# DJjjjhao/FIRA-ICSE

Measured on NVIDIA H100. Metric: train_commits_per_sec, higher is better.
Workload: dtype bf16

## Files before the change

fira_icse_b200/csrc/gcn_fused.cu:

```cuda
#include "tc_common.cuh"
#include "fira_b200.h"

namespace {

using namespace tc;

constexpr int D = 256;
constexpr int TM = 128;
constexpr int N_CONSUMER = 256;
constexpr int N_GATHER = 4;
constexpr int THREADS = N_CONSUMER + N_GATHER * 32;
constexpr int EC = 1024;
constexpr uint32_t B_BYTES = D * D * 2;
constexpr uint32_t A_BYTES = TM * D * 2;
constexpr uint32_t OFF_A = B_BYTES, OFF_ROWPTR = OFF_A + A_BYTES, OFF_COL = OFF_ROWPTR + 544, OFF_VAL = OFF_COL + EC * 4,
                   OFF_RS = OFF_VAL + EC * 4, SMEM_BYTES = OFF_RS + 4 * TM * 4;
constexpr int GATHER_BAR = 1;

struct Params {
  const int* rowptr; const int* col; const float* val;
  const __nv_bfloat16* x;
  long R;
  const float* bias; const float* c1; const float* gamma; const float* beta;
  __nv_bfloat16* z; __nv_bfloat16* outA; __nv_bfloat16* outB; long split;
  float* mean; float* rstd;
  float p_drop; uint64_t seed; const uint64_t* seed_ctr; uint32_t stream_id;
  const __nv_bfloat16* addend; __nv_bfloat16* agg_out; __nv_bfloat16* y;
};

__device__ __forceinline__ void tile_range(long R, int cta, int ncta, int t, long& r0, int& rows, int& ntiles) {
  const long rpc = (R + ncta - 1) / ncta;
  const long lo = (long)cta * rpc;
  const long hi = lo + rpc < R ? lo + rpc : R;
  const long n = hi > lo ? hi - lo : 0;
  ntiles = (int)((n + TM - 1) / TM);
  if (ntiles == 0) { r0 = 0; rows = 0; return; }
  long chunk = (n + ntiles - 1) / ntiles;
  chunk = (chunk + 7) & ~7L;
  if (chunk > TM) chunk = TM;
  r0 = lo + (long)t * chunk;
  const long e = r0 + chunk < hi ? r0 + chunk : hi;
  rows = (int)(e > r0 ? e - r0 : 0);
}

__device__ __forceinline__ uint4 pack8(const float* v) {
  uint4 r;
  __nv_bfloat162* h = reinterpret_cast<__nv_bfloat162*>(&r);
#pragma unroll
  for (int i = 0; i < 4; ++i) h[i] = __floats2bfloat162_rn(v[2 * i], v[2 * i + 1]);
  return r;
}
__device__ __forceinline__ void unpack8(const uint4& raw, float* v) {
  const __nv_bfloat162* h = reinterpret_cast<const __nv_bfloat162*>(&raw);
#pragma unroll
  for (int i = 0; i < 4; ++i) { const float2 f = __bfloat1622float2(h[i]); v[2 * i] = f.x; v[2 * i + 1] = f.y; }
}

template <int MODE>
__global__ void __launch_bounds__(THREADS, 1) gcn_fused_kernel(const __grid_constant__ CUtensorMap tmW, Params p) {
  extern __shared__ unsigned char smem_raw[];
  __shared__ __align__(8) unsigned long long b_full, a_full, a_empty;
  const uint32_t base = (smem_addr(smem_raw) + 1023u) & ~1023u;
  unsigned char* sm = smem_raw + (base - smem_addr(smem_raw));
  const int warp = threadIdx.x >> 5, lane = threadIdx.x & 31;
  const int cta = blockIdx.x, ncta = gridDim.x;
  long r0_; int rows_, ntiles;
  tile_range(p.R, cta, ncta, 0, r0_, rows_, ntiles);

  if (threadIdx.x == 0) {
    mbar_init(smem_addr(&b_full), 1);
    mbar_init(smem_addr(&a_full), N_GATHER * 32);
    mbar_init(smem_addr(&a_empty), N_CONSUMER);
    mbar_init_fence();
    tma_prefetch_desc(&tmW);
  }
  __syncthreads();
  pdl_wait(); pdl_trigger();

  if (warp >= N_CONSUMER / 32) {
    const int gw = warp - N_CONSUMER / 32;
    const int gtid = gw * 32 + lane;
    const int q = lane >> 3, ql = lane & 7;
    int* s_rowptr = reinterpret_cast<int*>(sm + OFF_ROWPTR);
    int* s_col = reinterpret_cast<int*>(sm + OFF_COL);
    float* s_val = reinterpret_cast<float*>(sm + OFF_VAL);
    float* s_rs = reinterpret_cast<float*>(sm + OFF_RS);
    for (int t = 0; t < ntiles; ++t) {
      long r0; int rows, nt_;
      tile_range(p.R, cta, ncta, t, r0, rows, nt_);
      if (t >= 1) named_bar(GATHER_BAR, N_GATHER * 32);
      for (int i = gtid; i <= rows; i += N_GATHER * 32) s_rowptr[i] = p.rowptr[r0 + i];
      named_bar(GATHER_BAR, N_GATHER * 32);
      const int e_lo = s_rowptr[0], e_hi = s_rowptr[rows];
      const int nE = e_hi - e_lo;
      const bool staged = nE <= EC;
      if (staged)
        for (int i = gtid; i < nE; i += N_GATHER * 32) { s_col[i] = p.col[e_lo + i]; s_val[i] = p.val[e_lo + i]; }
      if (t >= 1 && gtid == 0) mbar_wait(smem_addr(&a_empty), (t - 1) & 1);
      named_bar(GATHER_BAR, N_GATHER * 32);
      const int* cp = staged ? s_col : p.col + e_lo;
      const float* vp = staged ? s_val : p.val + e_lo;
#pragma unroll 1
      for (int it = 0; it < 8; ++it) {
        const int r = gw * 32 + it * 4 + q;
        if (r < rows) {
          const int e0 = s_rowptr[r] - e_lo, e1 = s_rowptr[r + 1] - e_lo;
          float acc[4][8];
#pragma unroll
          for (int j = 0; j < 4; ++j)
#pragma unroll
            for (int i = 0; i < 8; ++i) acc[j][i] = 0.f;
          float rsum = 0.f;
          int e = e0;
          for (; e + 1 < e1; e += 2) {
            const int c0 = cp[e], c1 = cp[e + 1];
            const float w0 = vp[e], w1 = vp[e + 1];
            const uint4* s0 = reinterpret_cast<const uint4*>(p.x + (long)c0 * D + ql * 8);
            const uint4* s1 = reinterpret_cast<const uint4*>(p.x + (long)c1 * D + ql * 8);
            uint4 a[4], b[4];
#pragma unroll
            for (int j = 0; j < 4; ++j) a[j] = __ldg(s0 + j * 8);
#pragma unroll
            for (int j = 0; j < 4; ++j) b[j] = __ldg(s1 + j * 8);
            rsum += w0 + w1;
#pragma unroll
            for (int j = 0; j < 4; ++j) {
              float f[8];
              unpack8(a[j], f);
#pragma unroll
              for (int i = 0; i < 8; ++i) acc[j][i] = fmaf(w0, f[i], acc[j][i]);
              unpack8(b[j], f);
#pragma unroll
              for (int i = 0; i < 8; ++i) acc[j][i] = fmaf(w1, f[i], acc[j][i]);
            }
          }
          if (e < e1) {
            const int c0 = cp[e];
            const float w0 = vp[e];
            const uint4* s0 = reinterpret_cast<const uint4*>(p.x + (long)c0 * D + ql * 8);
            uint4 a[4];
#pragma unroll
            for (int j = 0; j < 4; ++j) a[j] = __ldg(s0 + j * 8);
            rsum += w0;
#pragma unroll
            for (int j = 0; j < 4; ++j) {
              float f[8];
              unpack8(a[j], f);
#pragma unroll
              for (int i = 0; i < 8; ++i) acc[j][i] = fmaf(w0, f[i], acc[j][i]);
            }
          }
#pragma unroll
          for (int j = 0; j < 4; ++j) {
            const uint4 v = pack8(acc[j]);
            *reinterpret_cast<uint4*>(sm + OFF_A + j * 16384 + sw128_offset(r, ql)) = v;
            if (MODE == 1) *reinterpret_cast<uint4*>(p.agg_out + (r0 + r) * D + j * 64 + ql * 8) = v;
          }
          if (MODE == 0 && ql == 0) s_rs[(t & 3) * TM + r] = rsum;
        }
      }
      fence_proxy_async();
      mbar_arrive(smem_addr(&a_full));
    }
    return;
  }

  const int wg = warp >> 2, q4 = lane & 3;
  if (threadIdx.x == 0 && ntiles > 0) {
    mbar_expect_tx(smem_addr(&b_full), B_BYTES);
#pragma unroll
    for (int kb = 0; kb < 4; ++kb) tma_load_2d(base + kb * 32768, &tmW, kb * 64, 0, smem_addr(&b_full));
  }
  if (ntiles > 0) mbar_wait(smem_addr(&b_full), 0);
  const float* s_rs = reinterpret_cast<const float*>(sm + OFF_RS);
  uint64_t seed = p.seed;
  if (MODE == 0 && p.seed_ctr) seed += *p.seed_ctr;
  const float keep_scale = (MODE == 0 && p.p_drop > 0.f) ? 1.f / (1.f - p.p_drop) : 1.f;
  const __nv_bfloat16* resid = MODE == 0 ? p.x : p.addend;
  for (int t = 0; t < ntiles; ++t) {
    long r0; int rows, nt_;
    tile_range(p.R, cta, ncta, t, r0, rows, nt_);
    float acc[D / 2];
#pragma unroll
    for (int i = 0; i < D / 2; ++i) acc[i] = 0.f;
    mbar_wait(smem_addr(&a_full), t & 1);
    wgmma_fence();
#pragma unroll
    for (int kb = 0; kb < 4; ++kb)
#pragma unroll
      for (int k = 0; k < 4; ++k)
        wgmma<D, 0, 0>(acc, make_desc(base + OFF_A + kb * 16384 + wg * 8192 + k * 32, 16, 1024),
                       make_desc(base + kb * 32768 + k * 32, 16, 1024));
    wgmma_commit();
    wgmma_wait<0>();
    reg_fence<D / 2>(acc);
    mbar_arrive(smem_addr(&a_empty));
    int tr[2];
    bool live[2];
    long grow[2];
    float rs[2], sum[2] = {0.f, 0.f}, sq[2] = {0.f, 0.f};
#pragma unroll
    for (int h = 0; h < 2; ++h) {
      tr[h] = wg * 64 + (warp & 3) * 16 + (lane >> 2) + 8 * h;
      live[h] = tr[h] < rows;
      grow[h] = r0 + tr[h];
      rs[h] = (MODE == 0 && live[h]) ? s_rs[(t & 3) * TM + tr[h]] : 0.f;
    }
#pragma unroll
    for (int j = 0; j < D / 8; ++j) {
      const int c = 8 * j + 2 * q4;
      float2 bv = make_float2(0.f, 0.f), cv = make_float2(0.f, 0.f);
      if (MODE == 0) {
        bv = __ldg(reinterpret_cast<const float2*>(p.bias + c));
        cv = __ldg(reinterpret_cast<const float2*>(p.c1 + c));
      }
#pragma unroll
      for (int h = 0; h < 2; ++h) {
        float2 hv = make_float2(0.f, 0.f);
        if (live[h] && resid != nullptr) hv = __bfloat1622float2(__ldg(reinterpret_cast<const __nv_bfloat162*>(resid + grow[h] * D + c)));
        float v0 = acc[4 * j + 2 * h], v1 = acc[4 * j + 2 * h + 1];
        if (MODE == 0) {
          v0 = fmaf(rs[h], cv.x, v0 + bv.x);
          v1 = fmaf(rs[h], cv.y, v1 + bv.y);
          const __nv_bfloat162 zb = __floats2bfloat162_rn(v0, v1);
          if (live[h]) *reinterpret_cast<__nv_bfloat162*>(p.z + grow[h] * D + c) = zb;
          const float2 zf = __bfloat1622float2(zb);
          v0 = zf.x; v1 = zf.y;
          if (p.p_drop > 0.f) {
            const uint32_t m = dropout_keep8(seed, p.stream_id, (uint64_t)grow[h] * 32 + j, p.p_drop) >> (2 * q4);
            v0 = (m & 1) ? v0 * keep_scale : 0.f;
            v1 = (m & 2) ? v1 * keep_scale : 0.f;
          }
          v0 += hv.x; v1 += hv.y;
          acc[4 * j + 2 * h] = v0; acc[4 * j + 2 * h + 1] = v1;
          sum[h] += v0 + v1;
          sq[h] = fmaf(v0, v0, fmaf(v1, v1, sq[h]));
        } else if (live[h]) {
          *reinterpret_cast<__nv_bfloat162*>(p.y + grow[h] * D + c) = __floats2bfloat162_rn(v0 + hv.x, v1 + hv.y);
        }
      }
    }
    if (MODE == 0) {
      float mean[2], rstd[2];
#pragma unroll
      for (int h = 0; h < 2; ++h) {
        sum[h] += __shfl_xor_sync(0xffffffffu, sum[h], 1);
        sum[h] += __shfl_xor_sync(0xffffffffu, sum[h], 2);
        sq[h] += __shfl_xor_sync(0xffffffffu, sq[h], 1);
        sq[h] += __shfl_xor_sync(0xffffffffu, sq[h], 2);
        mean[h] = sum[h] * (1.f / D);
        const float var = fmaxf(sq[h] * (1.f / D) - mean[h] * mean[h], 0.f);
        rstd[h] = rsqrtf(var + kLnEps);
        if (live[h] && q4 == 0 && p.mean) { p.mean[grow[h]] = mean[h]; p.rstd[grow[h]] = rstd[h]; }
      }
#pragma unroll
      for (int j = 0; j < D / 8; ++j) {
        const int c = 8 * j + 2 * q4;
        const float2 gv = __ldg(reinterpret_cast<const float2*>(p.gamma + c));
        const float2 bt = __ldg(reinterpret_cast<const float2*>(p.beta + c));
#pragma unroll
        for (int h = 0; h < 2; ++h) {
          if (!live[h]) continue;
          const float o0 = fmaf((acc[4 * j + 2 * h] - mean[h]) * rstd[h], gv.x, bt.x);
          const float o1 = fmaf((acc[4 * j + 2 * h + 1] - mean[h]) * rstd[h], gv.y, bt.y);
          __nv_bfloat16* dst = grow[h] < p.split ? p.outA : p.outB;
          *reinterpret_cast<__nv_bfloat162*>(dst + grow[h] * D + c) = __floats2bfloat162_rn(o0, o1);
        }
      }
    }
  }
}

struct Segs { int B, n0, n1, n2; };
__device__ __forceinline__ long seg_row(const Segs& s, int b, int j) {
  if (j < s.n0) return (long)b * s.n0 + j;
  if (j < s.n0 + s.n1) return (long)s.B * s.n0 + (long)b * s.n1 + (j - s.n0);
  return (long)s.B * (s.n0 + s.n1) + (long)b * s.n2 + (j - s.n0 - s.n1);
}
__device__ __forceinline__ void seg_unrow(const Segs& s, long r, int& b, int& i) {
  const long e0 = (long)s.B * s.n0, e1 = e0 + (long)s.B * s.n1;
  if (r < e0) { b = (int)(r / s.n0); i = (int)(r % s.n0); }
  else if (r < e1) { long q = r - e0; b = (int)(q / s.n1); i = s.n0 + (int)(q % s.n1); }
// ... 35 lines not shown
    const int excl = carry + (warp ? warp_tot[warp - 1] : 0) + x - v;
    if (i < n) out[i] = excl;
    __syncthreads();
    if (threadIdx.x == 1023) carry = excl + v;
    __syncthreads();
  }
  if (threadIdx.x == 0) out[n] = carry;
}

__global__ void rows_fill_kernel(const int* __restrict__ rowptr, const int* __restrict__ col, const float* __restrict__ val,
                                 Segs s, int N, const int* __restrict__ rowptr_g, int* __restrict__ col_g,
                                 float* __restrict__ val_g) {
  pdl_wait(); pdl_trigger();
  const long R = (long)s.B * N;
  const int lane = threadIdx.x & 31;
  for (long r = (long)blockIdx.x * (blockDim.x >> 5) + (threadIdx.x >> 5); r < R; r += (long)gridDim.x * (blockDim.x >> 5)) {
    int b, i; seg_unrow(s, r, b, i);
    const long g = (long)b * N + i;
    const int e0 = rowptr[g], n = rowptr[g + 1] - e0, o0 = rowptr_g[r];
    for (int k = lane; k < n; k += 32) { col_g[o0 + k] = (int)seg_row(s, b, col[e0 + k]); val_g[o0 + k] = val[e0 + k]; }
  }
}

int launch_fused(int mode, const CUtensorMap& tm, const Params& p, cudaStream_t st) {
  static_assert(SMEM_BYTES + 1024 <= 227 * 1024, "fused GCN kernel: shared-memory budget");
  const size_t smem = SMEM_BYTES + 1024;
  cudaError_t e = mode == 0
      ? cudaFuncSetAttribute(gcn_fused_kernel<0>, cudaFuncAttributeMaxDynamicSharedMemorySize, (int)smem)
      : cudaFuncSetAttribute(gcn_fused_kernel<1>, cudaFuncAttributeMaxDynamicSharedMemorySize, (int)smem);
  if (e != cudaSuccess) { fira_set_error(FIRA_ERR_CUDA, "gcn_layer attr: %s", cudaGetErrorString(e)); return FIRA_ERR_CUDA; }
  long want = (p.R + 31) / 32;
  const int grid = (int)(want < fira_num_sms() ? (want < 1 ? 1 : want) : fira_num_sms());
  if (mode == 0) launch_k(gcn_fused_kernel<0>, dim3(grid), dim3(THREADS), smem, st, tm, p);
  else launch_k(gcn_fused_kernel<1>, dim3(grid), dim3(THREADS), smem, st, tm, p);
  return FIRA_OK;
}

}

extern "C" {

int fira_csr_to_rows(const int* rowptr, const int* col, const float* val, int B, int n_code, int n_sub, int n_ast,
                     int* counts, int* rowptr_rows, int* col_rows, float* val_rows, void* stream) {
  FIRA_CHECK_ARG(rowptr && col && val && counts && rowptr_rows && col_rows && val_rows, FIRA_ERR_ARG, "csr_to_rows: null");
  FIRA_CHECK_ARG(B > 0 && n_code > 0 && n_sub >= 0 && n_ast >= 0, FIRA_ERR_SHAPE, "csr_to_rows: segments");
  Segs s{B, n_code, n_sub, n_ast};
  const int N = n_code + n_sub + n_ast;
  const long R = (long)B * N;
  cudaStream_t st = (cudaStream_t)stream;
  int grid = (int)((R + 255) / 256 < fira_num_sms() * 4 ? (R + 255) / 256 : fira_num_sms() * 4);
  launch_k(rows_count_kernel, dim3(grid), dim3(256), 0, st, rowptr, s, N, counts);
  launch_k(rows_scan_kernel, dim3(1), dim3(1024), 0, st, counts, rowptr_rows, R);
  grid = (int)((R + 7) / 8 < fira_num_sms() * 8 ? (R + 7) / 8 : fira_num_sms() * 8);
  launch_k(rows_fill_kernel, dim3(grid), dim3(256), 0, st, rowptr, col, val, s, N, rowptr_rows, col_rows, val_rows);
  FIRA_CHECK_LAUNCH("fira_csr_to_rows");
  return FIRA_OK;
}

int fira_gcn_layer_fwd(const int* rowptr_rows, const int* col_rows, const float* val_rows, const void* h,
                       const void* w_merged, const float* bias, const float* c1, const float* gamma, const float* beta,
                       void* z, void* outA, void* outB, long split, float* mean, float* rstd, long rows, int dim,
                       float p_drop, uint64_t seed, const uint64_t* seed_ctr, uint32_t stream_id, void* stream) {
  FIRA_CHECK_ARG(dim == D, FIRA_ERR_SHAPE, "gcn_layer_fwd: dim %d != 256", dim);
  FIRA_CHECK_ARG(rows > 0, FIRA_ERR_SHAPE, "gcn_layer_fwd: rows %ld", rows);
  FIRA_CHECK_ARG(rowptr_rows && col_rows && val_rows && h && w_merged && bias && c1 && gamma && beta && z && outA && outB,
                 FIRA_ERR_ARG, "gcn_layer_fwd: null argument");
  FIRA_CHECK_ARG(fira_aligned16(h) && fira_aligned16(w_merged) && fira_aligned16(z) && fira_aligned16(outA) &&
                     fira_aligned16(outB) && fira_aligned16(bias) && fira_aligned16(c1) && fira_aligned16(gamma) &&
                     fira_aligned16(beta), FIRA_ERR_ALIGN, "gcn_layer_fwd: 16-B alignment");
  FIRA_CHECK_ARG(p_drop >= 0.f && p_drop < 1.f, FIRA_ERR_ARG, "gcn_layer_fwd: p_drop %f", p_drop);
  CUtensorMap tm;
  int rc = make_map_bf16(&tm, w_merged, D, D, D, 64, D, "gcn_layer_fwd");
  if (rc) return rc;
  Params p{};
  p.rowptr = rowptr_rows; p.col = col_rows; p.val = val_rows; p.x = (const __nv_bfloat16*)h; p.R = rows;
  p.bias = bias; p.c1 = c1; p.gamma = gamma; p.beta = beta;
  p.z = (__nv_bfloat16*)z; p.outA = (__nv_bfloat16*)outA; p.outB = (__nv_bfloat16*)outB; p.split = split;
  p.mean = mean; p.rstd = rstd; p.p_drop = p_drop; p.seed = seed; p.seed_ctr = seed_ctr; p.stream_id = stream_id;
  if ((rc = launch_fused(0, tm, p, (cudaStream_t)stream))) return rc;
  FIRA_CHECK_LAUNCH("fira_gcn_layer_fwd");
  return FIRA_OK;
}

int fira_gcn_layer_bwd(const int* rowptr_rows_t, const int* col_rows_t, const float* val_rows_t, const void* d_z,
                       const void* w_merged_t, const void* d_resid, void* agg_dz, void* d_h, long rows, int dim,
                       void* stream) {
  FIRA_CHECK_ARG(dim == D, FIRA_ERR_SHAPE, "gcn_layer_bwd: dim %d != 256", dim);
  FIRA_CHECK_ARG(rows > 0, FIRA_ERR_SHAPE, "gcn_layer_bwd: rows %ld", rows);
  FIRA_CHECK_ARG(rowptr_rows_t && col_rows_t && val_rows_t && d_z && w_merged_t && agg_dz && d_h, FIRA_ERR_ARG,
                 "gcn_layer_bwd: null argument");
  FIRA_CHECK_ARG(fira_aligned16(d_z) && fira_aligned16(w_merged_t) && fira_aligned16(d_resid) && fira_aligned16(agg_dz) &&
                     fira_aligned16(d_h), FIRA_ERR_ALIGN, "gcn_layer_bwd: 16-B alignment");
  CUtensorMap tm;
  int rc = make_map_bf16(&tm, w_merged_t, D, D, D, 64, D, "gcn_layer_bwd");
  if (rc) return rc;
  Params p{};
  p.rowptr = rowptr_rows_t; p.col = col_rows_t; p.val = val_rows_t; p.x = (const __nv_bfloat16*)d_z; p.R = rows;
  p.addend = (const __nv_bfloat16*)d_resid; p.agg_out = (__nv_bfloat16*)agg_dz; p.y = (__nv_bfloat16*)d_h;
  if ((rc = launch_fused(1, tm, p, (cudaStream_t)stream))) return rc;
  FIRA_CHECK_LAUNCH("fira_gcn_layer_bwd");
  return FIRA_OK;
}

}
```

fira_icse_b200/ops.py:

```python
import ctypes
import os

import torch

from . import _lib
from . import optim as _optim
from ._lib import FIRA_BF16, FIRA_F32, call

D = 256

if hasattr(torch.autograd.graph, "set_warn_on_accumulate_grad_stream_mismatch"):
    torch.autograd.graph.set_warn_on_accumulate_grad_stream_mismatch(False)


def _stream():
    return torch.cuda.current_stream().cuda_stream


def _ptr(t, off=0):
    if t is None:
        return None
    return t.data_ptr() + off * t.element_size()


# ... 224 lines not shown
            lane = _TURN[0]
            _TURN[0] += 1
        self.side = self.sides[lane % len(self.sides)]
        self.side.wait_stream(self.main)
        self.used.add(self.side)
        return torch.cuda.stream(self.side)

    def join(self):
        for s in self.used:
            self.main.wait_stream(s)
        self.used.clear()
        self.keep.clear()


class Prefetch:

    def __init__(self):
        self.wcache = {}
        self.items = None
        self.event = None
        self.layer_table = None


def _prep_encoder_layer(pr, fork, mark_emb, Wq, bq, Wk, bk, Wv, bv, Wo, W1, b1, W2, fused=True):
    f32 = dict(dtype=torch.float32, device=Wq.device)

    def done():
        ev = torch.cuda.Event()
        ev.record()
        return ev
    with fork(mark_emb, Wq, bq, Wk, bk, Wv, bv, Wo):
        Wqk = _optim.cat_rows((Wq, Wk))
        bqk = _optim.cat_rows((bq, bk))
        Vtab = linear(mark_emb, Wv, bv)
        for w in (Wqk, Wo):
            pr.w(w)
        ev_comb = done()
    with fork(W1, W2):
        Wc = torch.empty((D, D), **f32)
        gemm_raw(_ptr(W2), D, 1, _ptr(W1), D, 0, _ptr(Wc), D, D, D, D, splits=MERGE_SPLITS if pr.bf16 else 1)
        pr.w(Wc)
        WcT16 = Wc.t().contiguous().to(torch.bfloat16) if (pr.bf16 and fused) else None
        ev_wc = done()
    with fork(W2, b1):
        c1 = torch.empty((D,), **f32)
        gemm_raw(_ptr(W2), D, 1, _ptr(b1), D, 1, _ptr(c1), 1, D, 1, D, splits=1)
        ev_c1 = done()
    return (Wqk, bqk, Vtab, Wc, c1, WcT16), (ev_comb, ev_wc, ev_c1)


def prefetch_decoder(bf16, lp, device):
    pf = Prefetch()
    pr = Prec(bf16, pf.wcache)
    L = len(lp) // DEC_LAYER_PARAMS
    fork = Fork(device)
    with fork(*lp):
        Wkv = _optim.cat_rows([t for i in range(L) for t in (lp[i * 26 + 12], lp[i * 26 + 14])])
        bkv = _optim.cat_rows([t for i in range(L) for t in (lp[i * 26 + 13], lp[i * 26 + 15])])
        pr.w(Wkv)
        layers = []
        for i in range(L):
            q = lp[i * 26:(i + 1) * 26]
            Wqkv = _optim.cat_rows((q[0], q[2], q[4]))
            bqkv = _optim.cat_rows((q[1], q[3], q[5]))
            for w in (Wqkv, q[6], q[10], q[16], q[20], q[22]):
                pr.w(w)
            layers.append((Wqkv, bqkv))
        if bf16:
            ptrs = []
            for i in range(L):
                q = lp[i * 26:(i + 1) * 26]
# ... 45 lines not shown
        p_gcn = cfg["p_gcn"] if training else 0.0
        heads = cfg["heads"]
        pr = Prec(cfg.get("bf16", False), seed_ctr=cfg.get("seed_ctr"))
        dev = emb.device
        f32 = dict(dtype=torch.float32, device=dev)
        st = _stream()

        Xc = pr.empty((Mc, D), dev)
        Gin = pr.empty((R, D), dev)
        if cfg.get("pos") is not None:
            call("fira_embed_nodes_pos_fwd", _ptr(sou), _ptr(cfg["pos"]), _ptr(sub_token), _ptr(ast_change), _ptr(emb),
                 _ptr(ast_emb), _ptr(pos_table), _ptr(Xc), _ptr(Gin), B, n_code, n_sub, n_ast, D, pr.code, st)
        else:
            call("fira_embed_nodes_fwd", _ptr(sou), _ptr(sub_token), _ptr(ast_change), _ptr(emb), _ptr(ast_emb),
                 _ptr(pos_table), _ptr(Xc), _ptr(Gin), B, n_code, n_sub, n_ast, D, pr.code, st)
        fused = pr.bf16 and os.environ.get("FIRA_GCN_FUSED", "0") != "0"
        rs = None if fused else edges.rowsum(n_code, n_sub, n_ast)
        erows = edges.rows_csr(n_code, n_sub, n_ast) if fused else None
        saved = []
        fork = Fork(dev)
        preps, events = [], []
        for i in range(L):
            Wq, bq, Wk, bk, Wv, bv, Wo, bo, clw, clb, W1, b1, W2, b2, glw, glb = lp[i * 16:(i + 1) * 16]
            t, e = _prep_encoder_layer(pr, fork, mark_emb, Wq, bq, Wk, bk, Wv, bv, Wo, W1, b1, W2, fused=fused)
            preps.append(t)
            events.append(e)
        for i in range(L):
            Wq, bq, Wk, bk, Wv, bv, Wo, bo, clw, clb, W1, b1, W2, b2, glw, glb = lp[i * 16:(i + 1) * 16]
            sid = cfg["stream_base"] + i * 8
            cur = torch.cuda.current_stream()
            cur.wait_event(events[i][0])
            Wqk, bqk, Vtab, Wc, c1, WcT16 = preps[i]
            QK = pr.linear(Xc, Wqk, bqk)
            Cd = pr.empty((Mc, D), dev)
            call("fira_comb_gate_fwd", _ptr(QK), 2 * D, _ptr(Vtab), _ptr(mark), _ptr(Cd), Mc, D, D // heads,
                 float(p_comb), seed, _ptr(pr.seed_ctr), sid + 0, pr.code, st)
            Zc, st_c = pr.linear_ln(Cd, Wo, bo, Xc, clw, clb, Gin, Gin, Mc, Mc, p_comb, seed, sid + 1)
            Xc_n = pr.empty((Mc, D), dev)
            Gin_n = pr.empty((R, D), dev)
            cur.wait_event(events[i][1])
            cur.wait_event(events[i][2])
            if fused:
                G = None
                Z = pr.empty((R, D), dev)
                st_g = torch.empty((2, R), **f32)
                call("fira_gcn_layer_fwd", _ptr(erows[0]), _ptr(erows[1]), _ptr(erows[2]), _ptr(Gin), _ptr(pr.w(Wc)),
                     _ptr(b2), _ptr(c1), _ptr(glw), _ptr(glb), _ptr(Z), _ptr(Xc_n), _ptr(Gin_n), Mc, _ptr(st_g),
                     _ptr(st_g, R), R, D, float(p_gcn), seed, _ptr(pr.seed_ctr), sid + 2, st)
            else:
                G = pr.empty((R, D), dev)
                call("fira_gcn_aggregate", _ptr(edges.rowptr), _ptr(edges.col), _ptr(edges.val), _ptr(Gin), None,
                     _ptr(G), B, n_code, n_sub, n_ast, D, pr.code, st)
                Z, st_g = pr.linear_ln(G, Wc, b2, Gin, glw, glb, Xc_n, Gin_n, Mc, R, p_gcn, seed, sid + 2, rs=rs, rc=c1)
            saved.append((Xc, QK, Vtab, Cd, Zc, st_c, Gin, G, Z, st_g, Wqk, Wc, c1, WcT16))
            Xc, Gin = Xc_n, Gin_n
        memory = pr.empty((B, n_code + n_sub, D), dev)
        call("fira_pack_memory", _ptr(Xc), _ptr(Gin), _ptr(memory), B, n_code, n_sub, D, pr.code, st)
        fork.join()

        ctx.saved = saved
        ctx.wcache = pr.wcache
        ctx.misc = (cfg, sou, mark, ast_change, sub_token, edges, rs, B, n_code, n_sub, n_ast, p_comb, p_gcn, fused)
        ctx.save_for_backward(emb, ast_emb, mark_emb, *lp)
        return memory

    @staticmethod
    def backward(ctx, d_mem):
        cfg, sou, mark, ast_change, sub_token, edges, rs, B, n_code, n_sub, n_ast, p_comb, p_gcn, fused = ctx.misc
        emb, ast_emb, mark_emb, *lp = ctx.saved_tensors
        N = n_code + n_sub + n_ast
        R, Mc = B * N, B * n_code
        L = len(lp) // ENC_LAYER_PARAMS
        seed, heads = cfg["seed"], cfg["heads"]
        pr = Prec(cfg.get("bf16", False), ctx.wcache, seed_ctr=cfg.get("seed_ctr"))
        dev = emb.device
        f32 = dict(dtype=torch.float32, device=dev)
        st = _stream()
        et = edges.t()
        etrows = et.rows_csr(n_code, n_sub, n_ast) if fused else None
        d_mem = d_mem.contiguous().to(pr.tdt)
        dXc = pr.empty((Mc, D), dev)
        dGin = pr.empty((R, D), dev)
        call("fira_unpack_memory", _ptr(d_mem), _ptr(dXc), _ptr(dGin), B, n_code, n_sub, n_ast, D, pr.code, st)
        d_mark_emb = _gdest(mark_emb, tuple(mark_emb.shape), zero=True)
        grads = [None] * len(lp)
        fork = Fork(dev)
        for i in reversed(range(L)):
            Wq, bq, Wk, bk, Wv, bv, Wo, bo, clw, clb, W1, b1, W2, b2, glw, glb = lp[i * 16:(i + 1) * 16]
            Xc, QK, Vtab, Cd, Zc, st_c, Gin, G, Z, st_g, Wqk, Wc, c1, WcT16 = ctx.saved[i]
            sid = cfg["stream_base"] + i * 8
            dZ, dRes, d_glw, d_glb = pr.ln_bwd(dXc, dGin, Mc, Z, Gin, st_g, glw, R, p_gcn, seed, sid + 2, beta=glb)
            dGin_i = pr.empty((R, D), dev)
            if fused:
                AdZ = pr.empty((R, D), dev)
                call("fira_gcn_layer_bwd", _ptr(etrows[0]), _ptr(etrows[1]), _ptr(etrows[2]), _ptr(dZ), _ptr(WcT16),
                     _ptr(dRes), _ptr(AdZ), _ptr(dGin_i), R, D, st)
            with fork(dZ, G, rs, W1, W2, b1):
                d_b2 = _gdest(b2, (D,), zero=True)
                if fused:
                    fork.keep.append(AdZ)
                    colsum(dZ, D, R, D, out=d_b2)
                    d_c1 = torch.zeros(D, dtype=torch.float32, device=dev)
                    dWc = pr.linear_dw(AdZ, D, Gin, D, R, D, D, dbias=d_c1)
                else:
                    d_c1 = colsum(dZ, D, R, D, weight=rs)
                    dWc = pr.linear_dw(dZ, D, G, D, R, D, D, dbias=d_b2)
                ev_dwc = torch.cuda.Event()
                ev_dwc.record()
                fork.keep.extend((dWc, d_c1))
            with fork():
                torch.cuda.current_stream().wait_event(ev_dwc)
                d_W2 = _gdest(W2, (D, D))
                gemm_raw(_ptr(dWc), D, 1, _ptr(W1), D, 1, _ptr(d_W2), D, D, D, D, rs=d_c1, rc=b1, splits=MERGE_SPLITS if pr.bf16 else 1)
            with fork():
                torch.cuda.current_stream().wait_event(ev_dwc)
                d_W1 = _gdest(W1, (D, D))
                gemm_raw(_ptr(W2), D, 0, _ptr(dWc), D, 0, _ptr(d_W1), D, D, D, D, splits=MERGE_SPLITS if pr.bf16 else 1)
                d_b1 = _gdest(b1, (D,))
                gemm_raw(_ptr(W2), D, 0, _ptr(d_c1), 1, 0, _ptr(d_b1), 1, D, 1, D, splits=1)
# ... 435 lines not shown
```

include/fira_b200.h:

```cpp
#ifndef FIRA_B200_H_
#define FIRA_B200_H_

#include <stdint.h>

#ifdef __cplusplus
extern "C" {
#endif

#define FIRA_F32 0
#define FIRA_BF16 1
#define FIRA_EDGE_F32 0
#define FIRA_EDGE_BF16 1
#define FIRA_EDGE_F64 2

int fira_version(void);
const char* fira_last_error_string(void);
int fira_built_arch(void);
int fira_num_sms(void);
int fira_set_pdl(int on);
int fira_get_pdl(void);

int fira_gemm_f32(const float* A, long lda, int a_kcontig, const float* B, long ldb, int b_kcontig, float* C,
                  long ldc, int M, int N, int K, const float* bias, const float* rs, const float* rc, int relu,
                  int accumulate, int splits, void* stream);
// ... 61 lines not shown
int fira_pack_memory(const void* code, const void* rest, void* mem, int B, int n_code, int n_sub, int dim, int dtype,
                     void* stream);
int fira_unpack_memory(const void* d_mem, void* d_code, void* d_rest, int B, int n_code, int n_sub, int n_ast, int dim,
                       int dtype, void* stream);

int fira_csr_count_dense(const void* edge, int edge_dtype, long stride_b, long stride_i, long stride_j, int B, int N,
                         int* counts, int* rowptr, void* stream);
int fira_csr_fill_dense(const void* edge, int edge_dtype, long stride_b, long stride_i, long stride_j, int B, int N,
                        const int* rowptr, int* col, float* val, void* stream);
int fira_csr_rowsum(const int* rowptr, const float* val, int B, int n_code, int n_sub, int n_ast, float* out,
                    void* stream);
int fira_gcn_aggregate(const int* rowptr, const int* col, const float* val, const void* x, const void* addend,
                       void* y, int B, int n_code, int n_sub, int n_ast, int dim, int dtype, void* stream);

int fira_csr_to_rows(const int* rowptr, const int* col, const float* val, int B, int n_code, int n_sub, int n_ast,
                     int* counts, int* rowptr_rows, int* col_rows, float* val_rows, void* stream);
int fira_gcn_layer_fwd(const int* rowptr_rows, const int* col_rows, const float* val_rows, const void* h,
                       const void* w_merged, const float* bias, const float* c1, const float* gamma, const float* beta,
                       void* z, void* outA, void* outB, long split, float* mean, float* rstd, long rows, int dim,
                       float p_drop, uint64_t seed, const uint64_t* seed_ctr, uint32_t stream_id, void* stream);
int fira_gcn_layer_bwd(const int* rowptr_rows_t, const int* col_rows_t, const float* val_rows_t, const void* d_z,
                       const void* w_merged_t, const void* d_resid, void* agg_dz, void* d_h, long rows, int dim,
                       void* stream);

int fira_attn_fwd(const void* q, long ldq, const void* k, long ldk, const void* v, long ldv,
                  const unsigned char* key_mask, int causal, void* ctx, long ldo, float* stats, int B, int H, int Lq,
                  int Lk, int d_head, int dtype, void* stream);
int fira_attn_bwd(const void* q, long ldq, const void* k, long ldk, const void* v, long ldv,
                  const unsigned char* key_mask, int causal, const void* ctx, const void* d_ctx, long ldo,
                  const float* stats, void* dq, long lddq, void* dk, long lddk, void* dv, long lddv, int B, int H,
                  int Lq, int Lk, int d_head, int dtype, void* stream);

int fira_attn_packed_fwd(const void* q, long ldq, const void* k, long ldk, const void* v, long ldv, const int* ranges,
                         long kv_rows, const unsigned char* key_mask, int mask_pitch, int max_chunks, void* ctx, long ldo,
                         float* stats, int B, int H, int Lq, int d_head, int dtype, void* stream);
int fira_attn_packed_bwd(const void* q, long ldq, const void* k, long ldk, const void* v, long ldv, const int* ranges,
                         long kv_rows, const unsigned char* key_mask, int mask_pitch, int max_chunks, const void* ctx,
                         const void* d_ctx, long ldo, const float* stats, void* dq, long lddq, void* dk, long lddk,
                         void* dv, long lddv, int B, int H, int Lq, int d_head, int dtype, void* stream);
int fira_attn_bwd_rows(const void* q, long ldq, const void* k, long ldk, const void* v, long ldv, const int* ranges,
                       const unsigned char* key_mask, int mask_pitch, int causal, const int* qoff, long rows,
                       const void* ctx, const void* d_ctx, long ldo, const float* stats, void* dq, long lddq, void* dk,
                       long lddk, void* dv, long lddv, int B, int H, int Lq, int d_head, int dtype, void* stream);

int fira_decoder_fwd(const int* tar, const float* dec_emb, const float* pos_table, const unsigned char* tar_mask,
                     const void* kv, long ldkv, const unsigned char* mem_mask, const int* ranges, int S,
// ... 160 lines not shown
```

Baseline: 22490.

## Double-buffer fused GCN kernel, split N across warpgroups, drop transposed weight copy

Rewrites the fused GCN aggregate+GEMM+LayerNorm kernel to use 64-row tiles with two shared-memory A buffers, so gathering the next tile overlaps the current wgmma. Each consumer warpgroup now computes half the output columns for all rows, with row sums for LayerNorm combined across warpgroups through shared memory. Other changes: more gather warps, register reallocation via setmaxnreg, bias/gamma/beta cached in shared memory, residual prefetched before the MMA, dropout masks computed once and shared by shuffle, and a two-pass variance. The backward pass now reads the untransposed merged weight through a transposed-B wgmma path, which removes the per-step transpose and cast of Wc in Python. The cost is extra named barriers per tile and more complex synchronisation.

```diff
diff --git a/fira_icse_b200/csrc/gcn_fused.cu b/fira_icse_b200/csrc/gcn_fused.cu
--- a/fira_icse_b200/csrc/gcn_fused.cu
+++ b/fira_icse_b200/csrc/gcn_fused.cu
@@ -6,16 +6,19 @@
 using namespace tc;
 
 constexpr int D = 256;
-constexpr int TM = 128;
+constexpr int TM = 64;
+constexpr int NW = D / 2;
 constexpr int N_CONSUMER = 256;
-constexpr int N_GATHER = 4;
+constexpr int N_GATHER = 8;
 constexpr int THREADS = N_CONSUMER + N_GATHER * 32;
 constexpr int EC = 1024;
 constexpr uint32_t B_BYTES = D * D * 2;
 constexpr uint32_t A_BYTES = TM * D * 2;
-constexpr uint32_t OFF_A = B_BYTES, OFF_ROWPTR = OFF_A + A_BYTES, OFF_COL = OFF_ROWPTR + 544, OFF_VAL = OFF_COL + EC * 4,
-                   OFF_RS = OFF_VAL + EC * 4, SMEM_BYTES = OFF_RS + 4 * TM * 4;
+constexpr uint32_t OFF_A = B_BYTES, OFF_ROWPTR = OFF_A + 2 * A_BYTES, OFF_COL = OFF_ROWPTR + 512,
+                   OFF_VAL = OFF_COL + EC * 4, OFF_RS = OFF_VAL + EC * 4, OFF_RED = OFF_RS + 2 * TM * 4,
+                   OFF_CST = OFF_RED + 4 * TM * 4, SMEM_BYTES = OFF_CST + 4 * D * 4;
 constexpr int GATHER_BAR = 1;
+constexpr int CONSUMER_BAR = 2;
 
 struct Params {
   const int* rowptr; const int* col; const float* val;
@@ -28,19 +31,12 @@
   const __nv_bfloat16* addend; __nv_bfloat16* agg_out; __nv_bfloat16* y;
 };
 
-__device__ __forceinline__ void tile_range(long R, int cta, int ncta, int t, long& r0, int& rows, int& ntiles) {
-  const long rpc = (R + ncta - 1) / ncta;
-  const long lo = (long)cta * rpc;
-  const long hi = lo + rpc < R ? lo + rpc : R;
-  const long n = hi > lo ? hi - lo : 0;
-  ntiles = (int)((n + TM - 1) / TM);
-  if (ntiles == 0) { r0 = 0; rows = 0; return; }
-  long chunk = (n + ntiles - 1) / ntiles;
-  chunk = (chunk + 7) & ~7L;
-  if (chunk > TM) chunk = TM;
-  r0 = lo + (long)t * chunk;
-  const long e = r0 + chunk < hi ? r0 + chunk : hi;
-  rows = (int)(e > r0 ? e - r0 : 0);
+__device__ __forceinline__ void cta_rows(long R, long& lo, int& n, int& ntiles, int& chunk) {
+  lo = R * blockIdx.x / gridDim.x;
+  n = (int)(R * (blockIdx.x + 1) / gridDim.x - lo);
+  ntiles = (n + TM - 1) / TM;
+  if (ntiles == 1 && n > 16) ntiles = 2;
+  chunk = ntiles ? (n + ntiles - 1) / ntiles : 0;
 }
 
 __device__ __forceinline__ uint4 pack8(const float* v) {
@@ -56,21 +52,35 @@
   for (int i = 0; i < 4; ++i) { const float2 f = __bfloat1622float2(h[i]); v[2 * i] = f.x; v[2 * i + 1] = f.y; }
 }
 
-template <int MODE>
+__device__ __forceinline__ void row_sum2(float* v, float* red, int wg, const int* tr, int q4) {
+#pragma unroll
+  for (int h = 0; h < 2; ++h) {
+    v[h] += __shfl_xor_sync(0xffffffffu, v[h], 1);
+    v[h] += __shfl_xor_sync(0xffffffffu, v[h], 2);
+    if (q4 == 0) red[wg * TM + tr[h]] = v[h];
+  }
+  named_bar(CONSUMER_BAR, N_CONSUMER);
+#pragma unroll
+  for (int h = 0; h < 2; ++h) v[h] = red[tr[h]] + red[TM + tr[h]];
+}
+
+template <int MODE, int TB>
 __global__ void __launch_bounds__(THREADS, 1) gcn_fused_kernel(const __grid_constant__ CUtensorMap tmW, Params p) {
   extern __shared__ unsigned char smem_raw[];
-  __shared__ __align__(8) unsigned long long b_full, a_full, a_empty;
+  __shared__ __align__(8) unsigned long long b_full, a_full[2], a_empty[2];
   const uint32_t base = (smem_addr(smem_raw) + 1023u) & ~1023u;
   unsigned char* sm = smem_raw + (base - smem_addr(smem_raw));
   const int warp = threadIdx.x >> 5, lane = threadIdx.x & 31;
-  const int cta = blockIdx.x, ncta = gridDim.x;
-  long r0_; int rows_, ntiles;
-  tile_range(p.R, cta, ncta, 0, r0_, rows_, ntiles);
+  long lo;
+  int n_rows, ntiles, chunk;
+  cta_rows(p.R, lo, n_rows, ntiles, chunk);
 
   if (threadIdx.x == 0) {
     mbar_init(smem_addr(&b_full), 1);
-    mbar_init(smem_addr(&a_full), N_GATHER * 32);
-    mbar_init(smem_addr(&a_empty), N_CONSUMER);
+    for (int b = 0; b < 2; ++b) {
+      mbar_init(smem_addr(&a_full[b]), N_GATHER * 32);
+      mbar_init(smem_addr(&a_empty[b]), N_CONSUMER);
+    }
     mbar_init_fence();
     tma_prefetch_desc(&tmW);
   }
@@ -78,6 +88,7 @@
   pdl_wait(); pdl_trigger();
 
   if (warp >= N_CONSUMER / 32) {
+    asm volatile("setmaxnreg.dec.sync.aligned.u32 88;\n" ::: "memory");
     const int gw = warp - N_CONSUMER / 32;
     const int gtid = gw * 32 + lane;
     const int q = lane >> 3, ql = lane & 7;
@@ -85,31 +96,32 @@
     int* s_col = reinterpret_cast<int*>(sm + OFF_COL);
     float* s_val = reinterpret_cast<float*>(sm + OFF_VAL);
     float* s_rs = reinterpret_cast<float*>(sm + OFF_RS);
-    for (int t = 0; t < ntiles; ++t) {
-      long r0; int rows, nt_;
-      tile_range(p.R, cta, ncta, t, r0, rows, nt_);
-      if (t >= 1) named_bar(GATHER_BAR, N_GATHER * 32);
-      for (int i = gtid; i <= rows; i += N_GATHER * 32) s_rowptr[i] = p.rowptr[r0 + i];
+    for (int i = 0; i < ntiles; ++i) {
+      const int buf = i & 1;
+      const long r0 = lo + (long)i * chunk;
+      const int rows = min(chunk, n_rows - i * chunk);
+      if (i >= 1) named_bar(GATHER_BAR, N_GATHER * 32);
+      for (int k = gtid; k <= rows; k += N_GATHER * 32) s_rowptr[k] = p.rowptr[r0 + k];
       named_bar(GATHER_BAR, N_GATHER * 32);
       const int e_lo = s_rowptr[0], e_hi = s_rowptr[rows];
       const int nE = e_hi - e_lo;
       const bool staged = nE <= EC;
       if (staged)
-        for (int i = gtid; i < nE; i += N_GATHER * 32) { s_col[i] = p.col[e_lo + i]; s_val[i] = p.val[e_lo + i]; }
-      if (t >= 1 && gtid == 0) mbar_wait(smem_addr(&a_empty), (t - 1) & 1);
+        for (int k = gtid; k < nE; k += N_GATHER * 32) { s_col[k] = p.col[e_lo + k]; s_val[k] = p.val[e_lo + k]; }
+      if (i >= 2 && gtid == 0) mbar_wait(smem_addr(&a_empty[buf]), ((i - 2) >> 1) & 1);
       named_bar(GATHER_BAR, N_GATHER * 32);
       const int* cp = staged ? s_col : p.col + e_lo;
       const float* vp = staged ? s_val : p.val + e_lo;
+      unsigned char* sa = sm + OFF_A + buf * A_BYTES;
 #pragma unroll 1
-      for (int it = 0; it < 8; ++it) {
-        const int r = gw * 32 + it * 4 + q;
-        if (r < rows) {
+      for (int r = gw * 4 + q; r < rows; r += N_GATHER * 4) {
+        {
           const int e0 = s_rowptr[r] - e_lo, e1 = s_rowptr[r + 1] - e_lo;
           float acc[4][8];
 #pragma unroll
           for (int j = 0; j < 4; ++j)
 #pragma unroll
-            for (int i = 0; i < 8; ++i) acc[j][i] = 0.f;
+            for (int k = 0; k < 8; ++k) acc[j][k] = 0.f;
           float rsum = 0.f;
           int e = e0;
           for (; e + 1 < e1; e += 2) {
@@ -128,10 +140,10 @@
               float f[8];
               unpack8(a[j], f);
 #pragma unroll
-              for (int i = 0; i < 8; ++i) acc[j][i] = fmaf(w0, f[i], acc[j][i]);
+              for (int k = 0; k < 8; ++k) acc[j][k] = fmaf(w0, f[k], acc[j][k]);
               unpack8(b[j], f);
 #pragma unroll
-              for (int i = 0; i < 8; ++i) acc[j][i] = fmaf(w1, f[i], acc[j][i]);
+              for (int k = 0; k < 8; ++k) acc[j][k] = fmaf(w1, f[k], acc[j][k]);
             }
           }
           if (e < e1) {
@@ -147,77 +159,114 @@
               float f[8];
               unpack8(a[j], f);
 #pragma unroll
-              for (int i = 0; i < 8; ++i) acc[j][i] = fmaf(w0, f[i], acc[j][i]);
+              for (int k = 0; k < 8; ++k) acc[j][k] = fmaf(w0, f[k], acc[j][k]);
             }
           }
 #pragma unroll
           for (int j = 0; j < 4; ++j) {
             const uint4 v = pack8(acc[j]);
-            *reinterpret_cast<uint4*>(sm + OFF_A + j * 16384 + sw128_offset(r, ql)) = v;
+            *reinterpret_cast<uint4*>(sa + j * (TM * 128) + sw128_offset(r, ql)) = v;
             if (MODE == 1) *reinterpret_cast<uint4*>(p.agg_out + (r0 + r) * D + j * 64 + ql * 8) = v;
           }
-          if (MODE == 0 && ql == 0) s_rs[(t & 3) * TM + r] = rsum;
+          if (MODE == 0 && ql == 0) s_rs[buf * TM + r] = rsum;
         }
       }
       fence_proxy_async();
-      mbar_arrive(smem_addr(&a_full));
+      mbar_arrive(smem_addr(&a_full[buf]));
     }
     return;
   }
 
+  asm volatile("setmaxnreg.inc.sync.aligned.u32 168;\n" ::: "memory");
   const int wg = warp >> 2, q4 = lane & 3;
   if (threadIdx.x == 0 && ntiles > 0) {
     mbar_expect_tx(smem_addr(&b_full), B_BYTES);
-#pragma unroll
-    for (int kb = 0; kb < 4; ++kb) tma_load_2d(base + kb * 32768, &tmW, kb * 64, 0, smem_addr(&b_full));
+    if (TB == 0) {
+#pragma unroll
+      for (int kb = 0; kb < 4; ++kb) tma_load_2d(base + kb * 32768, &tmW, kb * 64, 0, smem_addr(&b_full));
+    } else {
+#pragma unroll
+      for (int kb = 0; kb < 4; ++kb)
+#pragma unroll
+        for (int np = 0; np < 4; ++np) tma_load_2d(base + kb * 32768 + np * 8192, &tmW, np * 64, kb * 64, smem_addr(&b_full));
+    }
   }
   if (ntiles > 0) mbar_wait(smem_addr(&b_full), 0);
   const float* s_rs = reinterpret_cast<const float*>(sm + OFF_RS);
+  float* s_red = reinterpret_cast<float*>(sm + OFF_RED);
+  float* s_cst = reinterpret_cast<float*>(sm + OFF_CST);
+  if (MODE == 0) {
+    for (int k = threadIdx.x; k < D; k += N_CONSUMER) {
+      s_cst[k] = p.bias[k]; s_cst[D + k] = p.c1[k]; s_cst[2 * D + k] = p.gamma[k]; s_cst[3 * D + k] = p.beta[k];
+    }
+    named_bar(CONSUMER_BAR, N_CONSUMER);
+  }
   uint64_t seed = p.seed;
   if (MODE == 0 && p.seed_ctr) seed += *p.seed_ctr;
   const float keep_scale = (MODE == 0 && p.p_drop > 0.f) ? 1.f / (1.f - p.p_drop) : 1.f;
   const __nv_bfloat16* resid = MODE == 0 ? p.x : p.addend;
-  for (int t = 0; t < ntiles; ++t) {
-    long r0; int rows, nt_;
-    tile_range(p.R, cta, ncta, t, r0, rows, nt_);
-    float acc[D / 2];
-#pragma unroll
-    for (int i = 0; i < D / 2; ++i) acc[i] = 0.f;
-    mbar_wait(smem_addr(&a_full), t & 1);
+  const int n0 = wg * NW;
+  int tr[2];
+#pragma unroll
+  for (int h = 0; h < 2; ++h) tr[h] = (warp & 3) * 16 + (lane >> 2) + 8 * h;
+  for (int i = 0; i < ntiles; ++i) {
+    const int buf = i & 1;
+    const long r0 = lo + (long)i * chunk;
+    const int rows = min(chunk, n_rows - i * chunk);
+    bool live[2];
+    long grow[2];
+#pragma unroll
+    for (int h = 0; h < 2; ++h) {
+      live[h] = tr[h] < rows;
+      grow[h] = r0 + tr[h];
+    }
+    __nv_bfloat162 hres[NW / 8][2];
+#pragma unroll
+    for (int j = 0; j < NW / 8; ++j)
+#pragma unroll
+      for (int h = 0; h < 2; ++h)
+        hres[j][h] = (live[h] && resid != nullptr)
+                         ? __ldg(reinterpret_cast<const __nv_bfloat162*>(resid + grow[h] * D + n0 + 8 * j + 2 * q4))
+                         : __floats2bfloat162_rn(0.f, 0.f);
+    float acc[NW / 2];
+#pragma unroll
+    for (int k = 0; k < NW / 2; ++k) acc[k] = 0.f;
+    mbar_wait(smem_addr(&a_full[buf]), (i >> 1) & 1);
+    float rs[2];
+#pragma unroll
+    for (int h = 0; h < 2; ++h) rs[h] = (MODE == 0 && live[h]) ? s_rs[buf * TM + tr[h]] : 0.f;
     wgmma_fence();
+    const uint32_t sa = base + OFF_A + buf * A_BYTES;
 #pragma unroll
     for (int kb = 0; kb < 4; ++kb)
 #pragma unroll
-      for (int k = 0; k < 4; ++k)
-        wgmma<D, 0, 0>(acc, make_desc(base + OFF_A + kb * 16384 + wg * 8192 + k * 32, 16, 1024),
-                       make_desc(base + kb * 32768 + k * 32, 16, 1024));
+      for (int k = 0; k < 4; ++k) {
+        const uint64_t da = make_desc(sa + kb * (TM * 128) + k * 32, 16, 1024);
+        const uint64_t db = TB == 0 ? make_desc(base + kb * 32768 + n0 * 128 + k * 32, 16, 1024)
+                                      : make_desc(base + kb * 32768 + (n0 / 64) * 8192 + k * 2048, 8192, 1024);
+        wgmma<NW, 0, TB>(acc, da, db);
+      }
     wgmma_commit();
     wgmma_wait<0>();
-    reg_fence<D / 2>(acc);
-    mbar_arrive(smem_addr(&a_empty));
-    int tr[2];
-    bool live[2];
-    long grow[2];
-    float rs[2], sum[2] = {0.f, 0.f}, sq[2] = {0.f, 0.f};
-#pragma unroll
-    for (int h = 0; h < 2; ++h) {
-      tr[h] = wg * 64 + (warp & 3) * 16 + (lane >> 2) + 8 * h;
-      live[h] = tr[h] < rows;
-      grow[h] = r0 + tr[h];
-      rs[h] = (MODE == 0 && live[h]) ? s_rs[(t & 3) * TM + tr[h]] : 0.f;
-    }
-#pragma unroll
-    for (int j = 0; j < D / 8; ++j) {
-      const int c = 8 * j + 2 * q4;
+    reg_fence<NW / 2>(acc);
+    mbar_arrive(smem_addr(&a_empty[buf]));
+    float sum[2] = {0.f, 0.f};
+    uint32_t mask[2] = {0u, 0u};
+#pragma unroll
+    for (int j = 0; j < NW / 8; ++j) {
+      const int c = n0 + 8 * j + 2 * q4;
+      if (MODE == 0 && p.p_drop > 0.f && (j & 3) == 0)
+#pragma unroll
+        for (int h = 0; h < 2; ++h)
+          mask[h] = dropout_keep8(seed, p.stream_id, (uint64_t)grow[h] * 32 + ((n0 >> 3) + j + q4), p.p_drop);
       float2 bv = make_float2(0.f, 0.f), cv = make_float2(0.f, 0.f);
       if (MODE == 0) {
-        bv = __ldg(reinterpret_cast<const float2*>(p.bias + c));
-        cv = __ldg(reinterpret_cast<const float2*>(p.c1 + c));
+        bv = *reinterpret_cast<const float2*>(s_cst + c);
+        cv = *reinterpret_cast<const float2*>(s_cst + D + c);
       }
 #pragma unroll
       for (int h = 0; h < 2; ++h) {
-        float2 hv = make_float2(0.f, 0.f);
-        if (live[h] && resid != nullptr) hv = __bfloat1622float2(__ldg(reinterpret_cast<const __nv_bfloat162*>(resid + grow[h] * D + c)));
+        const float2 hv = __bfloat1622float2(hres[j][h]);
         float v0 = acc[4 * j + 2 * h], v1 = acc[4 * j + 2 * h + 1];
         if (MODE == 0) {
           v0 = fmaf(rs[h], cv.x, v0 + bv.x);
@@ -227,37 +276,41 @@
           const float2 zf = __bfloat1622float2(zb);
           v0 = zf.x; v1 = zf.y;
           if (p.p_drop > 0.f) {
-            const uint32_t m = dropout_keep8(seed, p.stream_id, (uint64_t)grow[h] * 32 + j, p.p_drop) >> (2 * q4);
+            const uint32_t m = __shfl_sync(0xffffffffu, mask[h], (lane & ~3) | (j & 3)) >> (2 * q4);
             v0 = (m & 1) ? v0 * keep_scale : 0.f;
             v1 = (m & 2) ? v1 * keep_scale : 0.f;
           }
           v0 += hv.x; v1 += hv.y;
           acc[4 * j + 2 * h] = v0; acc[4 * j + 2 * h + 1] = v1;
           sum[h] += v0 + v1;
-          sq[h] = fmaf(v0, v0, fmaf(v1, v1, sq[h]));
         } else if (live[h]) {
           *reinterpret_cast<__nv_bfloat162*>(p.y + grow[h] * D + c) = __floats2bfloat162_rn(v0 + hv.x, v1 + hv.y);
         }
       }
     }
     if (MODE == 0) {
-      float mean[2], rstd[2];
+      float mean[2], rstd[2], sq[2] = {0.f, 0.f};
+      row_sum2(sum, s_red, wg, tr, q4);
+#pragma unroll
+      for (int h = 0; h < 2; ++h) mean[h] = sum[h] * (1.f / D);
+#pragma unroll
+      for (int j = 0; j < NW / 8; ++j)
+#pragma unroll
+        for (int h = 0; h < 2; ++h) {
+          const float d0 = acc[4 * j + 2 * h] - mean[h], d1 = acc[4 * j + 2 * h + 1] - mean[h];
+          sq[h] = fmaf(d0, d0, fmaf(d1, d1, sq[h]));
+        }
+      row_sum2(sq, s_red + 2 * TM, wg, tr, q4);
 #pragma unroll
       for (int h = 0; h < 2; ++h) {
-        sum[h] += __shfl_xor_sync(0xffffffffu, sum[h], 1);
-        sum[h] += __shfl_xor_sync(0xffffffffu, sum[h], 2);
-        sq[h] += __shfl_xor_sync(0xffffffffu, sq[h], 1);
-        sq[h] += __shfl_xor_sync(0xffffffffu, sq[h], 2);
-        mean[h] = sum[h] * (1.f / D);
-        const float var = fmaxf(sq[h] * (1.f / D) - mean[h] * mean[h], 0.f);
-        rstd[h] = rsqrtf(var + kLnEps);
-        if (live[h] && q4 == 0 && p.mean) { p.mean[grow[h]] = mean[h]; p.rstd[grow[h]] = rstd[h]; }
-      }
-#pragma unroll
-      for (int j = 0; j < D / 8; ++j) {
-        const int c = 8 * j + 2 * q4;
-        const float2 gv = __ldg(reinterpret_cast<const float2*>(p.gamma + c));
-        const float2 bt = __ldg(reinterpret_cast<const float2*>(p.beta + c));
+        rstd[h] = rsqrtf(sq[h] * (1.f / D) + kLnEps);
+        if (live[h] && wg == 0 && q4 == 0 && p.mean) { p.mean[grow[h]] = mean[h]; p.rstd[grow[h]] = rstd[h]; }
+      }
+#pragma unroll
+      for (int j = 0; j < NW / 8; ++j) {
+        const int c = n0 + 8 * j + 2 * q4;
+        const float2 gv = *reinterpret_cast<const float2*>(s_cst + 2 * D + c);
+        const float2 bt = *reinterpret_cast<const float2*>(s_cst + 3 * D + c);
 #pragma unroll
         for (int h = 0; h < 2; ++h) {
           if (!live[h]) continue;
@@ -339,17 +392,34 @@
   }
 }
 
-int launch_fused(int mode, const CUtensorMap& tm, const Params& p, cudaStream_t st) {
+template <int MODE, int TB>
+int launch_fused(const CUtensorMap& tm, const Params& p, cudaStream_t st) {
   static_assert(SMEM_BYTES + 1024 <= 227 * 1024, "fused GCN kernel: shared-memory budget");
   const size_t smem = SMEM_BYTES + 1024;
-  cudaError_t e = mode == 0
-      ? cudaFuncSetAttribute(gcn_fused_kernel<0>, cudaFuncAttributeMaxDynamicSharedMemorySize, (int)smem)
-      : cudaFuncSetAttribute(gcn_fused_kernel<1>, cudaFuncAttributeMaxDynamicSharedMemorySize, (int)smem);
+  cudaError_t e = cudaFuncSetAttribute(gcn_fused_kernel<MODE, TB>, cudaFuncAttributeMaxDynamicSharedMemorySize, (int)smem);
   if (e != cudaSuccess) { fira_set_error(FIRA_ERR_CUDA, "gcn_layer attr: %s", cudaGetErrorString(e)); return FIRA_ERR_CUDA; }
-  long want = (p.R + 31) / 32;
-  const int grid = (int)(want < fira_num_sms() ? (want < 1 ? 1 : want) : fira_num_sms());
-  if (mode == 0) launch_k(gcn_fused_kernel<0>, dim3(grid), dim3(THREADS), smem, st, tm, p);
-  else launch_k(gcn_fused_kernel<1>, dim3(grid), dim3(THREADS), smem, st, tm, p);
+  const long want = (p.R + 31) / 32;
+  const int grid = (int)(want < fira_num_sms() ? want : fira_num_sms());
+  launch_k(gcn_fused_kernel<MODE, TB>, dim3(grid), dim3(THREADS), smem, st, tm, p);
+  return FIRA_OK;
+}
+
+int gcn_layer_bwd(const int* rowptr, const int* col, const float* val, const void* d_z, const void* w, int transposed,
+                  const void* d_resid, void* agg_dz, void* d_h, long rows, int dim, void* stream) {
+  FIRA_CHECK_ARG(dim == D, FIRA_ERR_SHAPE, "gcn_layer_bwd: dim %d != 256", dim);
+  FIRA_CHECK_ARG(rows > 0, FIRA_ERR_SHAPE, "gcn_layer_bwd: rows %ld", rows);
+  FIRA_CHECK_ARG(rowptr && col && val && d_z && w && agg_dz && d_h, FIRA_ERR_ARG, "gcn_layer_bwd: null argument");
+  FIRA_CHECK_ARG(fira_aligned16(d_z) && fira_aligned16(w) && fira_aligned16(d_resid) && fira_aligned16(agg_dz) &&
+                     fira_aligned16(d_h), FIRA_ERR_ALIGN, "gcn_layer_bwd: 16-B alignment");
+  CUtensorMap tm;
+  int rc = make_map_bf16(&tm, w, D, D, D, 64, transposed ? D : 64, "gcn_layer_bwd");
+  if (rc) return rc;
+  Params p{};
+  p.rowptr = rowptr; p.col = col; p.val = val; p.x = (const __nv_bfloat16*)d_z; p.R = rows;
+  p.addend = (const __nv_bfloat16*)d_resid; p.agg_out = (__nv_bfloat16*)agg_dz; p.y = (__nv_bfloat16*)d_h;
+  if ((rc = transposed ? launch_fused<1, 0>(tm, p, (cudaStream_t)stream) : launch_fused<1, 1>(tm, p, (cudaStream_t)stream)))
+    return rc;
+  FIRA_CHECK_LAUNCH("fira_gcn_layer_bwd");
   return FIRA_OK;
 }
 
@@ -394,7 +464,7 @@
   p.bias = bias; p.c1 = c1; p.gamma = gamma; p.beta = beta;
   p.z = (__nv_bfloat16*)z; p.outA = (__nv_bfloat16*)outA; p.outB = (__nv_bfloat16*)outB; p.split = split;
   p.mean = mean; p.rstd = rstd; p.p_drop = p_drop; p.seed = seed; p.seed_ctr = seed_ctr; p.stream_id = stream_id;
-  if ((rc = launch_fused(0, tm, p, (cudaStream_t)stream))) return rc;
+  if ((rc = launch_fused<0, 0>(tm, p, (cudaStream_t)stream))) return rc;
   FIRA_CHECK_LAUNCH("fira_gcn_layer_fwd");
   return FIRA_OK;
 }
@@ -402,21 +472,13 @@
 int fira_gcn_layer_bwd(const int* rowptr_rows_t, const int* col_rows_t, const float* val_rows_t, const void* d_z,
                        const void* w_merged_t, const void* d_resid, void* agg_dz, void* d_h, long rows, int dim,
                        void* stream) {
-  FIRA_CHECK_ARG(dim == D, FIRA_ERR_SHAPE, "gcn_layer_bwd: dim %d != 256", dim);
-  FIRA_CHECK_ARG(rows > 0, FIRA_ERR_SHAPE, "gcn_layer_bwd: rows %ld", rows);
-  FIRA_CHECK_ARG(rowptr_rows_t && col_rows_t && val_rows_t && d_z && w_merged_t && agg_dz && d_h, FIRA_ERR_ARG,
-                 "gcn_layer_bwd: null argument");
-  FIRA_CHECK_ARG(fira_aligned16(d_z) && fira_aligned16(w_merged_t) && fira_aligned16(d_resid) && fira_aligned16(agg_dz) &&
-                     fira_aligned16(d_h), FIRA_ERR_ALIGN, "gcn_layer_bwd: 16-B alignment");
-  CUtensorMap tm;
-  int rc = make_map_bf16(&tm, w_merged_t, D, D, D, 64, D, "gcn_layer_bwd");
-  if (rc) return rc;
-  Params p{};
-  p.rowptr = rowptr_rows_t; p.col = col_rows_t; p.val = val_rows_t; p.x = (const __nv_bfloat16*)d_z; p.R = rows;
-  p.addend = (const __nv_bfloat16*)d_resid; p.agg_out = (__nv_bfloat16*)agg_dz; p.y = (__nv_bfloat16*)d_h;
-  if ((rc = launch_fused(1, tm, p, (cudaStream_t)stream))) return rc;
-  FIRA_CHECK_LAUNCH("fira_gcn_layer_bwd");
-  return FIRA_OK;
-}
-
-}
+  return gcn_layer_bwd(rowptr_rows_t, col_rows_t, val_rows_t, d_z, w_merged_t, 1, d_resid, agg_dz, d_h, rows, dim, stream);
+}
+
+int fira_gcn_layer_bwd_merged(const int* rowptr_rows_t, const int* col_rows_t, const float* val_rows_t, const void* d_z,
+                              const void* w_merged, const void* d_resid, void* agg_dz, void* d_h, long rows, int dim,
+                              void* stream) {
+  return gcn_layer_bwd(rowptr_rows_t, col_rows_t, val_rows_t, d_z, w_merged, 0, d_resid, agg_dz, d_h, rows, dim, stream);
+}
+
+}
diff --git a/fira_icse_b200/ops.py b/fira_icse_b200/ops.py
--- a/fira_icse_b200/ops.py
+++ b/fira_icse_b200/ops.py
@@ -270,7 +270,7 @@
         self.layer_table = None
 
 
-def _prep_encoder_layer(pr, fork, mark_emb, Wq, bq, Wk, bk, Wv, bv, Wo, W1, b1, W2, fused=True):
+def _prep_encoder_layer(pr, fork, mark_emb, Wq, bq, Wk, bk, Wv, bv, Wo, W1, b1, W2):
     f32 = dict(dtype=torch.float32, device=Wq.device)
 
     def done():
@@ -288,13 +288,12 @@
         Wc = torch.empty((D, D), **f32)
         gemm_raw(_ptr(W2), D, 1, _ptr(W1), D, 0, _ptr(Wc), D, D, D, D, splits=MERGE_SPLITS if pr.bf16 else 1)
         pr.w(Wc)
-        WcT16 = Wc.t().contiguous().to(torch.bfloat16) if (pr.bf16 and fused) else None
         ev_wc = done()
     with fork(W2, b1):
         c1 = torch.empty((D,), **f32)
         gemm_raw(_ptr(W2), D, 1, _ptr(b1), D, 1, _ptr(c1), 1, D, 1, D, splits=1)
         ev_c1 = done()
-    return (Wqk, bqk, Vtab, Wc, c1, WcT16), (ev_comb, ev_wc, ev_c1)
+    return (Wqk, bqk, Vtab, Wc, c1), (ev_comb, ev_wc, ev_c1)
 
 
 def prefetch_decoder(bf16, lp, device):
@@ -386,7 +385,7 @@
         preps, events = [], []
         for i in range(L):
             Wq, bq, Wk, bk, Wv, bv, Wo, bo, clw, clb, W1, b1, W2, b2, glw, glb = lp[i * 16:(i + 1) * 16]
-            t, e = _prep_encoder_layer(pr, fork, mark_emb, Wq, bq, Wk, bk, Wv, bv, Wo, W1, b1, W2, fused=fused)
+            t, e = _prep_encoder_layer(pr, fork, mark_emb, Wq, bq, Wk, bk, Wv, bv, Wo, W1, b1, W2)
             preps.append(t)
             events.append(e)
         for i in range(L):
@@ -394,7 +393,7 @@
             sid = cfg["stream_base"] + i * 8
             cur = torch.cuda.current_stream()
             cur.wait_event(events[i][0])
-            Wqk, bqk, Vtab, Wc, c1, WcT16 = preps[i]
+            Wqk, bqk, Vtab, Wc, c1 = preps[i]
             QK = pr.linear(Xc, Wqk, bqk)
             Cd = pr.empty((Mc, D), dev)
             call("fira_comb_gate_fwd", _ptr(QK), 2 * D, _ptr(Vtab), _ptr(mark), _ptr(Cd), Mc, D, D // heads,
@@ -416,7 +415,7 @@
                 call("fira_gcn_aggregate", _ptr(edges.rowptr), _ptr(edges.col), _ptr(edges.val), _ptr(Gin), None,
                      _ptr(G), B, n_code, n_sub, n_ast, D, pr.code, st)
                 Z, st_g = pr.linear_ln(G, Wc, b2, Gin, glw, glb, Xc_n, Gin_n, Mc, R, p_gcn, seed, sid + 2, rs=rs, rc=c1)
-            saved.append((Xc, QK, Vtab, Cd, Zc, st_c, Gin, G, Z, st_g, Wqk, Wc, c1, WcT16))
+            saved.append((Xc, QK, Vtab, Cd, Zc, st_c, Gin, G, Z, st_g, Wqk, Wc, c1))
             Xc, Gin = Xc_n, Gin_n
         memory = pr.empty((B, n_code + n_sub, D), dev)
         call("fira_pack_memory", _ptr(Xc), _ptr(Gin), _ptr(memory), B, n_code, n_sub, D, pr.code, st)
@@ -451,14 +450,14 @@
         fork = Fork(dev)
         for i in reversed(range(L)):
             Wq, bq, Wk, bk, Wv, bv, Wo, bo, clw, clb, W1, b1, W2, b2, glw, glb = lp[i * 16:(i + 1) * 16]
-            Xc, QK, Vtab, Cd, Zc, st_c, Gin, G, Z, st_g, Wqk, Wc, c1, WcT16 = ctx.saved[i]
+            Xc, QK, Vtab, Cd, Zc, st_c, Gin, G, Z, st_g, Wqk, Wc, c1 = ctx.saved[i]
             sid = cfg["stream_base"] + i * 8
             dZ, dRes, d_glw, d_glb = pr.ln_bwd(dXc, dGin, Mc, Z, Gin, st_g, glw, R, p_gcn, seed, sid + 2, beta=glb)
             dGin_i = pr.empty((R, D), dev)
             if fused:
                 AdZ = pr.empty((R, D), dev)
-                call("fira_gcn_layer_bwd", _ptr(etrows[0]), _ptr(etrows[1]), _ptr(etrows[2]), _ptr(dZ), _ptr(WcT16),
-                     _ptr(dRes), _ptr(AdZ), _ptr(dGin_i), R, D, st)
+                call("fira_gcn_layer_bwd_merged", _ptr(etrows[0]), _ptr(etrows[1]), _ptr(etrows[2]), _ptr(dZ),
+                     _ptr(pr.w(Wc)), _ptr(dRes), _ptr(AdZ), _ptr(dGin_i), R, D, st)
             with fork(dZ, G, rs, W1, W2, b1):
                 d_b2 = _gdest(b2, (D,), zero=True)
                 if fused:
diff --git a/include/fira_b200.h b/include/fira_b200.h
--- a/include/fira_b200.h
+++ b/include/fira_b200.h
@@ -107,6 +107,9 @@
 int fira_gcn_layer_bwd(const int* rowptr_rows_t, const int* col_rows_t, const float* val_rows_t, const void* d_z,
                        const void* w_merged_t, const void* d_resid, void* agg_dz, void* d_h, long rows, int dim,
                        void* stream);
+int fira_gcn_layer_bwd_merged(const int* rowptr_rows_t, const int* col_rows_t, const float* val_rows_t, const void* d_z,
+                              const void* w_merged, const void* d_resid, void* agg_dz, void* d_h, long rows, int dim,
+                              void* stream);
 
 int fira_attn_fwd(const void* q, long ldq, const void* k, long ldk, const void* v, long ldv,
                   const unsigned char* key_mask, int causal, void* ctx, long ldo, float* stats, int B, int H, int Lq,
```

Result: no change. 22420 (median of 6 runs) (-0.3%).
